# sjtuytc/betapose

Hardware: AMD Instinct MI355X
Metric: frames/sec (640x480, 50-kp KPD) (higher is better)
Workload: dtype f32 as an exact 3-way bf16 operand split (6 bf16 MFMA products), f32 accumulate and activations

## Files before the change

betapose_amd/_lib.py:

```python
from __future__ import annotations

import ctypes as C
import os
import threading

_HERE = os.path.dirname(os.path.abspath(__file__))
LIB_PATH = os.environ.get("BP_LIB") or os.path.join(_HERE, "libbetapose_hip.so")
_lock = threading.Lock()
_lib = None

c_float_p = C.POINTER(C.c_float)
c_double_p = C.POINTER(C.c_double)
c_int_p = C.POINTER(C.c_int)
vp = C.c_void_p

PROTOTYPES = {
    "bp_last_error": (C.c_char_p, []),
    "bp_version": (C.c_int, []),
    "bp_device_count": (C.c_int, []),
    "bp_device_name": (C.c_int, [C.c_int, C.c_char_p, C.c_int]),
    "bp_yolo_create": (C.c_int, [C.c_char_p, C.c_char_p, C.c_int, C.c_int, C.c_int, C.POINTER(vp)]),
    "bp_yolo_create_from_memory": (C.c_int, [C.c_char_p, vp, C.c_size_t, C.c_int, C.c_int, C.c_int, C.POINTER(vp)]),
    "bp_yolo_clone": (C.c_int, [vp, C.POINTER(vp)]),
    "bp_kpd_clone": (C.c_int, [vp, C.POINTER(vp)]),
    "bp_yolo_destroy": (None, [vp]),
    "bp_yolo_rows": (C.c_int, [vp]),
    "bp_yolo_attrs": (C.c_int, [vp]),
    "bp_yolo_forward": (C.c_int, [vp, vp, C.c_int, vp, vp]),
    "bp_yolo_forward_select": (C.c_int, [vp, vp, C.c_int, C.c_float, C.c_int, vp, vp, vp]),
    "bp_yolo_select": (C.c_int, [vp, C.c_int, C.c_int, C.c_int, C.c_float, C.c_int, vp, vp]),
    "bp_yolo_tap_count": (C.c_int, [vp]),
    "bp_yolo_tap_info": (C.c_int, [vp, C.c_int, C.c_char_p, C.c_int, c_int_p, c_int_p, c_int_p]),
    "bp_yolo_tap_copy": (C.c_int, [vp, C.c_int, C.c_int, vp, vp]),
    "bp_kpd_create": (C.c_int, [vp, C.c_size_t, C.c_int, C.c_int, C.c_int, C.POINTER(vp)]),
    "bp_kpd_destroy": (None, [vp]),
    "bp_kpd_forward": (C.c_int, [vp, vp, C.c_int, vp, vp]),
    "bp_kpd_forward_argmax": (C.c_int, [vp, vp, C.c_int, vp, vp, vp]),
    "bp_kpd_tap_count": (C.c_int, [vp]),
    "bp_kpd_tap_info": (C.c_int, [vp, C.c_int, C.c_char_p, C.c_int, c_int_p, c_int_p, c_int_p]),
    "bp_kpd_tap_copy": (C.c_int, [vp, C.c_int, C.c_int, vp, vp]),
    "bp_yolo_set_policy": (C.c_int, [vp, C.c_int, C.c_int, C.c_int, C.c_int]),
    "bp_kpd_set_policy": (C.c_int, [vp, C.c_int, C.c_int, C.c_int, C.c_int]),
    "bp_yolo_set_precision": (C.c_int, [vp, C.c_int]),
    "bp_kpd_set_precision": (C.c_int, [vp, C.c_int]),
    "bp_calibrate_ticks": (C.c_int, [C.c_longlong, c_float_p, vp]),
    "bp_yolo_set_prefetch": (C.c_int, [vp, C.c_int]),
    "bp_kpd_set_prefetch": (C.c_int, [vp, C.c_int]),
    "bp_yolo_set_fusion": (C.c_int, [vp, C.c_int]),
    "bp_kpd_set_fusion": (C.c_int, [vp, C.c_int]),
    "bp_yolo_fused_launches": (C.c_int, [vp, C.c_int, C.POINTER(C.c_int)]),
    "bp_kpd_fused_launches": (C.c_int, [vp, C.c_int, C.POINTER(C.c_int)]),
    "bp_yolo_xcd_errors": (C.c_int, [vp, C.POINTER(C.c_int), vp]),
    "bp_kpd_xcd_errors": (C.c_int, [vp, C.POINTER(C.c_int), vp]),
# ... 129 lines not shown
```

betapose_amd/csrc/aux_kernels.hip:

```cpp
#include "bp_common.h"

namespace bp {

__device__ __forceinline__ void store_plane(unsigned short* planes, long long idx, long long plane_elems, int np, float v) {
    if (np == 1) {
        const _Float16 h = (_Float16)v;
        planes[idx] = __builtin_bit_cast(unsigned short, h);
    } else if (np == 3) {
        const __bf16 h1 = (__bf16)v;
        const float r1 = v - (float)h1;
        const __bf16 h2 = (__bf16)r1;
        const __bf16 h3 = (__bf16)(r1 - (float)h2);
        planes[idx] = __builtin_bit_cast(unsigned short, h1);
        planes[idx + plane_elems] = __builtin_bit_cast(unsigned short, h2);
        planes[idx + 2 * plane_elems] = __builtin_bit_cast(unsigned short, h3);
    }
}

static inline int grid_for(long long n, int block = 256, int cap = 4096) {
    BP_CHECK(n < (1ll << 31), "tensor too large for 32-bit indexing");
    long long g = (n + block - 1) / block;
    return (int)(g < 1 ? 1 : (g > cap ? cap : g));
}

// ... 221 lines not shown
}

struct YoloHeads {
    YoloHead h[4];
    int n;
};
__device__ __forceinline__ float sigmoidf_(float x) { return 1.f / (1.f + expf(-x)); }

__global__ void yolo_decode_kernel(YoloHeads hs, int N, int reso, int attrs, int rows, float* __restrict__ pred) {
    const long long total = (long long)N * rows;
    for (int e = blockIdx.x * blockDim.x + threadIdx.x; e < (int)total; e += gridDim.x * blockDim.x) {
        const int row = (int)(e % rows);
        const int n = (int)(e / rows);
        int hi = 0;
        for (int k = 1; k < hs.n; ++k)
            if (row >= hs.h[k].row_off) hi = k;
        const YoloHead& H = hs.h[hi];
        const int g = H.g;
        const int r = row - H.row_off;
        const int a = r / (g * g);
        const int cell = r - a * g * g;
        const int gy = cell / g, gx = cell - gy * g;
        const float stride = (float)(reso / g);
        const float* t = H.t + ((long long)n * g * g + cell) * (3 * attrs) + a * attrs;
        float* o = pred + e * attrs;
        o[0] = (sigmoidf_(t[0]) + (float)gx) * stride;
        o[1] = (sigmoidf_(t[1]) + (float)gy) * stride;
        o[2] = (expf(t[2]) * (H.aw[a] / stride)) * stride;
        o[3] = (expf(t[3]) * (H.ah[a] / stride)) * stride;
        for (int k = 4; k < attrs; ++k) o[k] = sigmoidf_(t[k]);
    }
}
void launch_yolo_decode(const YoloHead* heads, int nheads, int N, int reso, int attrs, int rows, float* pred,
                        hipStream_t s) {
    BP_CHECK(nheads <= 4, "at most 4 yolo heads");
    YoloHeads hs;
    hs.n = nheads;
    for (int i = 0; i < nheads; ++i) hs.h[i] = heads[i];
    hipLaunchKernelGGL(yolo_decode_kernel, dim3(grid_for((long long)N * rows)), dim3(256), 0, s, hs, N, reso, attrs, rows, pred);
}

__global__ __launch_bounds__(1024) void yolo_select_kernel(const float* __restrict__ pred, int rows, int attrs,
                                                            float conf, int num_classes, float* __restrict__ sel, int sel_ld) {
    __shared__ float sv[16];
    __shared__ int si[16];
    const int n = blockIdx.x;
    const float* P = pred + (long long)n * rows * attrs;
// ... 24 lines not shown
            if (sv[k] > best || (sv[k] == best && si[k] < bi)) { best = sv[k]; bi = si[k]; }
        float* o = sel + (long long)n * sel_ld;
        if (best < 0.f) {
            o[0] = __int_as_float(-1);
            for (int k = 1; k < 8; ++k) o[k] = 0.f;
        } else {
            const float* q = P + (long long)bi * attrs;
            o[0] = __int_as_float(bi);
            o[1] = q[0] - q[2] / 2;
            o[2] = q[1] - q[3] / 2;
            o[3] = q[0] + q[2] / 2;
            o[4] = q[1] + q[3] / 2;
            o[5] = q[4];
            o[6] = q[5];
            o[7] = 0.f;
        }
    }
}
void launch_yolo_select(const float* pred, int N, int rows, int attrs, float conf, int num_classes, float* sel,
                        hipStream_t s, int sel_ld) {
    hipLaunchKernelGGL(yolo_select_kernel, dim3(N), dim3(1024), 0, s, pred, rows, attrs, conf, num_classes, sel, sel_ld);
}

__global__ __launch_bounds__(1024) void yolo_decode_select_kernel(YoloHeads hs, int reso, int attrs, int rows, float conf, int num_classes,
                                                                   float* __restrict__ sel, int sel_ld) {
    __shared__ float sv[16];
    __shared__ int si[16];
    const int n = blockIdx.x;
    const int ncls = min(num_classes, attrs - 5);
    auto locate = [&](int row, int* a) -> const float* {
        int hi = 0;
        for (int k = 1; k < hs.n; ++k)
            if (row >= hs.h[k].row_off) hi = k;
        const YoloHead& H = hs.h[hi];
        const int g = H.g, r = row - H.row_off;
        *a = r / (g * g);
        const int cell = r - *a * g * g;
        return H.t + ((long long)n * g * g + cell) * (3 * attrs) + *a * attrs;
    };
    float best = -1.f;
    int bi = 0x7fffffff;
    for (int r = threadIdx.x; r < rows; r += blockDim.x) {
        int a;
        const float* t = locate(r, &a);
        const float obj = sigmoidf_(t[4]);
        if (!(obj > conf)) continue;
        int cls = 0;
        float cm = sigmoidf_(t[5]);
        for (int k = 1; k < ncls; ++k) {
            const float v = sigmoidf_(t[5 + k]);
            if (v > cm) { cm = v; cls = k; }
        }
        if (cls != 0) continue;
        if (obj > best || (obj == best && r < bi)) { best = obj; bi = r; }
    }
    for (int off = 32; off > 0; off >>= 1) {
        const float ov = __shfl_down(best, off, 64);
        const int oi = __shfl_down(bi, off, 64);
        if (ov > best || (ov == best && oi < bi)) { best = ov; bi = oi; }
    }
    const int w = threadIdx.x >> 6;
    if ((threadIdx.x & 63) == 0) { sv[w] = best; si[w] = bi; }
    __syncthreads();
    if (threadIdx.x == 0) {
        for (int k = 1; k < (int)(blockDim.x >> 6); ++k)
            if (sv[k] > best || (sv[k] == best && si[k] < bi)) { best = sv[k]; bi = si[k]; }
        float* o = sel + (long long)n * sel_ld;
        if (best < 0.f) {
            o[0] = __int_as_float(-1);
            for (int k = 1; k < 8; ++k) o[k] = 0.f;
        } else {
            int a, hi = 0;
            const float* t = locate(bi, &a);
            for (int k = 1; k < hs.n; ++k)
                if (bi >= hs.h[k].row_off) hi = k;
            const YoloHead& H = hs.h[hi];
            const int g = H.g, r = bi - H.row_off, cell = r - a * g * g;
            const int gy = cell / g, gx = cell - gy * g;
            const float stride = (float)(reso / g);
            const float q0 = (sigmoidf_(t[0]) + (float)gx) * stride;
            const float q1 = (sigmoidf_(t[1]) + (float)gy) * stride;
            const float q2 = (expf(t[2]) * (H.aw[a] / stride)) * stride;
            const float q3 = (expf(t[3]) * (H.ah[a] / stride)) * stride;
            o[0] = __int_as_float(bi);
            o[1] = q0 - q2 / 2;
            o[2] = q1 - q3 / 2;
            o[3] = q0 + q2 / 2;
            o[4] = q1 + q3 / 2;
            o[5] = sigmoidf_(t[4]);
            o[6] = sigmoidf_(t[5]);
            o[7] = 0.f;
        }
    }
}
void launch_yolo_decode_select(const YoloHead* heads, int nheads, int N, int reso, int attrs, int rows, float conf, int num_classes,
                               float* sel, hipStream_t s, int sel_ld) {
    BP_CHECK(nheads <= 4, "at most 4 yolo heads");
    YoloHeads hs;
    hs.n = nheads;
    for (int i = 0; i < nheads; ++i) hs.h[i] = heads[i];
    hipLaunchKernelGGL(yolo_decode_select_kernel, dim3(N), dim3(1024), 0, s, hs, reso, attrs, rows, conf, num_classes, sel, sel_ld);
}

__global__ __launch_bounds__(256) void heatmap_argmax_kernel(const float* __restrict__ hm, int H, int W,
                                                              float* __restrict__ out, int C, int out_ld) {
    __shared__ float sv[4];
    __shared__ int si[4];
    const int HW = H * W;
    const float* P = hm + (long long)blockIdx.x * HW;
    float best = -INFINITY;
    int bi = 0x7fffffff;
    for (int i = threadIdx.x; i < HW; i += 256) {
        const float v = P[i];
        if (v > best) { best = v; bi = i; }
    }
    for (int off = 32; off > 0; off >>= 1) {
        const float ov = __shfl_down(best, off, 64);
        const int oi = __shfl_down(bi, off, 64);
        if (ov > best || (ov == best && oi < bi)) { best = ov; bi = oi; }
    }
    if ((threadIdx.x & 63) == 0) { sv[threadIdx.x >> 6] = best; si[threadIdx.x >> 6] = bi; }
    __syncthreads();
    if (threadIdx.x == 0) {
        for (int k = 1; k < 4; ++k)
// ... 261 lines not shown
```

betapose_amd/csrc/bp_common.h:

```cpp
#pragma once
#include <hip/hip_runtime.h>
#include <cstdint>
#include <cstdio>
#include <mutex>
#include <set>
#include <stdexcept>
#include <string>
#include <utility>

namespace bp {

struct Error : std::runtime_error {
    using std::runtime_error::runtime_error;
};

#define BP_HIP(expr)                                                                      \
    do {                                                                                  \
        hipError_t _e = (expr);                                                           \
        if (_e != hipSuccess)                                                             \
            throw ::bp::Error(std::string(#expr) + ": " + hipGetErrorString(_e) + " @" +  \
                              __FILE__ + ":" + std::to_string(__LINE__));                 \
    } while (0)

#define BP_CHECK(cond, msg)                                                               \
// ... 178 lines not shown
};

size_t mega_lds_bytes(const MegaOp& o);
void mega_make_conv_op(const ConvParams& p, int tile, MegaOp* out);
void launch_mega(const MegaArgs& a, size_t lds_bytes, hipStream_t s);

void launch_nchw_to_nhwc(const float* in, float* out, int N, int C, int H, int W, hipStream_t s);
void launch_nhwc_to_nchw(const float* in, int in_ld, float* out, int N, int C, int H, int W, hipStream_t s);
void launch_maxpool3s2p1(const float* in, float* out, int N, int H, int W, int C, int OH, int OW, hipStream_t s,
                         unsigned short* planes = nullptr, long long plane_elems = 0, int np = 0);
void launch_add(const float* a, int a_ld, const float* b, int b_ld, float* out, int out_ld,
                long long pixels, int C, hipStream_t s);
void launch_upsample2(const float* in, int in_ld, float* out, int out_ld, int N, int H, int W, int C, hipStream_t s);
void launch_copy_channels(const float* in, int in_ld, float* out, int out_ld, long long pixels, int C, hipStream_t s);
void launch_pixel_shuffle2(const float* in, float* out, int N, int H, int W, int C, hipStream_t s,
                           unsigned short* planes = nullptr, long long plane_elems = 0, int np = 0);
int avgpool_parts(int HW);
void launch_avgpool(const float* in, int in_ld, float* out, int N, int HW, int C, hipStream_t s);
void launch_fc(const float* in, const float* w, const float* bias, float* out, int N, int Cin, int Cout,
               int act, int in_parts, float in_scale, hipStream_t s);

struct YoloHead {
    const float* t;
    int g;
    float aw[3], ah[3];
    int row_off;
};
void launch_yolo_decode(const YoloHead* heads, int nheads, int N, int reso, int attrs, int rows,
                        float* pred, hipStream_t s);
void launch_yolo_select(const float* pred, int N, int rows, int attrs, float conf, int num_classes,
                        float* sel, hipStream_t s, int sel_ld = 8);
void launch_yolo_decode_select(const YoloHead* heads, int nheads, int N, int reso, int attrs, int rows, float conf, int num_classes,
                               float* sel, hipStream_t s, int sel_ld = 8);
void launch_heatmap_argmax(const float* hm, int N, int C, int H, int W, float* out, hipStream_t s, int out_ld = 0);

void launch_f32_to_f16(const float* in, unsigned short* out, long long n, hipStream_t s);
void launch_f32_to_bf16x3(const float* in, unsigned short* out_planes, long long n, hipStream_t s);
void launch_f32_to_f16_staged(const float* in, unsigned short* out, int CoutPad, int Kpad, hipStream_t s);
void launch_f32_to_bf16x3_staged(const float* in, unsigned short* out, int CoutPad, int Kpad, hipStream_t s, int Cin_pl = 0);
void launch_probe_placement(int* d_out, int blocks, hipStream_t s);
void launch_spin_ticks(long long ticks, hipStream_t s);

void launch_crop(const uint8_t* frames, int batch, int H, int W, const float* sel, int reso, const float* boxes,
                 float* out_nhwc, float* out_nchw, float* pts, int oh, int ow, hipStream_t s, int sel_ld = 8, int pts_ld = 8);

struct ResizeTables {
    const int* hb;
    const int* hk;
    int ksize_h;
    const int* vb;
    const int* vk;
    int ksize_v;
};
void launch_resize_bicubic(const uint8_t* in, int batch, int H, int W, uint8_t* tmp, float* out_nhwc, uint8_t* out_u8,
                           int oh, int ow, const ResizeTables& t, int swap_rb, hipStream_t s);

// ... 2 lines not shown
```

betapose_amd/csrc/c_api.cpp:

```cpp
#include "../../include/betapose_hip.h"

#include <algorithm>
#include <cmath>
#include <cstdlib>
#include <cstring>
#include <fstream>
#include <memory>
#include <sstream>
#include <vector>

#include "engine.h"
#include "frame_io.h"

namespace bp {
int solve_pnp(const double* P, const double* U, int n, const double* K, double* R, double* t);
int solve_pnp_refined(const double* P, const double* U, int n, const double* K, double* R, double* t);
int solve_pnp_ransac(const double* P, const double* U, int n, const double* K, double reproj_err, int max_trials,
                     double confidence, double* R, double* t, unsigned char* inlier_mask);
void pnp_ransac_samples(int n, int max_trials, int* idx);
void pnp_ransac_trials_needed(int n, double confidence, int* need);
int pose_nms(const float* bboxes, const float* bbox_scores, const float* preds, const float* scores, int n, int K,
             int* out_pick, float* out_pose, float* out_score, float* out_prop);
int pose_error_blocks(int n);
void launch_pose_errors(const double* model, int n, const double* gt, const double* est, int P, const double* K,
// ... 255 lines not shown
    y->net->forward(d_img, false, batch, d_pred, 0.f, 0, nullptr, (hipStream_t)stream);
    return 0;
    BP_CATCH
}
int bp_yolo_forward_select(bp_yolo* y, const float* d_img, int batch, float conf, int num_classes, float* d_pred,
                           float* d_sel, void* stream) {
    BP_TRY
    BP_CHECK(y && d_img && d_sel, "null argument");
    y->net->forward(d_img, false, batch, d_pred, conf, num_classes, d_sel, (hipStream_t)stream);
    return 0;
    BP_CATCH
}

int bp_yolo_select(const float* d_pred, int batch, int rows, int attrs, float conf, int num_classes, float* d_sel,
                   void* stream) {
    BP_TRY
    BP_CHECK(d_pred && d_sel && batch >= 1 && rows >= 1 && attrs >= 6, "bad argument");
    bp::launch_yolo_select(d_pred, batch, rows, attrs, conf, num_classes, d_sel, (hipStream_t)stream);
    BP_HIP(hipGetLastError());
    return 0;
    BP_CATCH
}

static int tap_info(const bp::Net& n, int i, char* name, int cap, int* C, int* H, int* W) {
    if (i < 0 || i >= n.tap_count()) { g_err = "tap index"; return -1; }
    if (name && cap > 0) std::snprintf(name, cap, "%s", n.tap_name(i));
    n.tap_shape(i, C, H, W);
    return 0;
}
int bp_yolo_tap_count(const bp_yolo* y) { return y ? y->net->tap_count() : -1; }
int bp_yolo_tap_info(const bp_yolo* y, int i, char* name, int cap, int* C, int* H, int* W) {
    if (!y || !C || !H || !W) { g_err = "null argument"; return -1; }
    return tap_info(*y->net, i, name, cap, C, H, W);
}
int bp_yolo_tap_copy(bp_yolo* y, int i, int batch, float* d_out, void* stream) {
    BP_TRY
    BP_CHECK(y && d_out, "null argument");
    y->net->tap_copy(i, batch, d_out, (hipStream_t)stream);
    return 0;
    BP_CATCH
}

int bp_kpd_create(const float* stream, size_t n_floats, int n_classes, int max_batch, int device, bp_kpd** out) {
    BP_TRY
    BP_CHECK(stream && out, "null argument");
    BP_HIP(hipSetDevice(device));
// ... 143 lines not shown
int bp_yolo_xcd_errors(bp_yolo* y, int* count, void* stream) {
    BP_TRY
    BP_CHECK(y && count, "null argument");
    BP_HIP(hipSetDevice(y->device));
    *count = y->net->take_xcd_errors((hipStream_t)stream);
    return 0;
    BP_CATCH
}
int bp_kpd_xcd_errors(bp_kpd* k, int* count, void* stream) {
    BP_TRY
    BP_CHECK(k && count, "null argument");
    BP_HIP(hipSetDevice(k->device));
    *count = k->net->take_xcd_errors((hipStream_t)stream);
    return 0;
    BP_CATCH
}
int bp_yolo_set_stamps(bp_yolo* y, unsigned long long* d_buf, int slots) { y->net->set_stamps(d_buf, slots); return 0; }
int bp_kpd_set_stamps(bp_kpd* k, unsigned long long* d_buf, int slots) { k->net->set_stamps(d_buf, slots); return 0; }
static int op_name(const bp::Net& net, int i, char* out, int cap) {
    if (i < 0 || i >= (int)net.ops().size() || !out || cap <= 0) return -1;
    const bp::Op& op = net.ops()[i];
    if (op.type == bp::OP_CONV)
        std::snprintf(out, (size_t)cap, "%s k%d %dx%d %d->%d s%d", net.op_name(i), op.conv.ksize, op.conv.OH, op.conv.OW, op.conv.Cin,
                      op.conv.Cout, op.conv.stride);
    else
        std::snprintf(out, (size_t)cap, "%s", net.op_name(i));
    return op.type == bp::OP_CONV ? 1 : 0;
}
int bp_yolo_op_name(const bp_yolo* y, int i, char* out, int cap) { return op_name(*y->net, i, out, cap); }
int bp_kpd_op_name(const bp_kpd* k, int i, char* out, int cap) { return op_name(*k->net, i, out, cap); }
size_t bp_yolo_device_bytes(const bp_yolo* y) { return y->net->device_bytes(); }
size_t bp_kpd_device_bytes(const bp_kpd* k) { return k->net->device_bytes(); }

int bp_crop(const uint8_t* d_frames, int batch, int H, int W, const float* d_sel, int reso, const float* d_boxes,
            float* d_out_nchw, float* d_out_nhwc, float* d_pts, int oh, int ow, void* stream) {
    BP_TRY
    BP_CHECK(d_frames && (d_sel || d_boxes) && (d_out_nchw || d_out_nhwc), "null argument");
    bp::launch_crop(d_frames, batch, H, W, d_sel, reso, d_boxes, d_out_nhwc, d_out_nchw, d_pts, oh, ow, (hipStream_t)stream);
    BP_HIP(hipGetLastError());
    return 0;
    BP_CATCH
}

int bp_resize_bicubic(const uint8_t* d_in, int batch, int H, int W, int oh, int ow, int swap_rb, uint8_t* d_out_u8,
                      float* d_out_nhwc, void* stream) {
    BP_TRY
    BP_CHECK(d_in && (d_out_u8 || d_out_nhwc), "null argument");
// ... 722 lines not shown
```

betapose_amd/csrc/engine.cpp:

```cpp
#include "engine.h"

#include <algorithm>
#include <cmath>
#include <cstdlib>
#include <cstring>
#include <sstream>

namespace bp {

Arena::~Arena() {
    for (void* p : ptrs_) (void)hipFree(p);
}
void* Arena::alloc_bytes(size_t bytes) {
    void* p = nullptr;
    bytes = (bytes + 255) & ~size_t(255);
    BP_HIP(hipMalloc(&p, bytes));
    ptrs_.push_back(p);
    total_ += bytes;
    return p;
}
float* Arena::alloc(size_t n) { return static_cast<float*>(alloc_bytes(n * sizeof(float))); }

Tensor Net::new_tensor(int H, int W, int C) {
    Tensor t;
// ... 556 lines not shown
        dB = upload_weights(B.data(), B.size());
    }

    Op op;
    op.type = OP_CONV;
    op.name = name;
    ConvParams& c = op.conv;
    c.in = in.p; c.in_ld = in.ld; c.N = 1; c.H = in.H; c.W = in.W; c.Cin = Cin;
    c.w = dW; c.Kpad = Kpad; c.Ktrue = K; c.bias = dB; c.cin_pack = cpk;
    c.out = out_view.p; c.out_ld = out_view.ld; c.OH = OH; c.OW = OW; c.Cout = Cout;
    c.ksize = k; c.stride = stride; c.pad = pad; c.act = act;
    c.res = res ? res->p : nullptr; c.res_ld = res ? res->ld : 0; c.res_scale = res_scale;
    c.res_after_act = res_after_act; c.store_mode = store_mode;
    c.M = OH * OW; c.nchunks = Kpad / 32; c.splits = 1; c.chunks_per_split = c.nchunks; c.partial = nullptr;
    c.tickets = nullptr;
    c.stamps = nullptr;
    c.w16 = nullptr; c.w16s = nullptr;
    c.in16 = nullptr; c.out16 = nullptr; c.wpl = nullptr; c.wbd = nullptr; c.in16_plane = c.out16_plane = 0; c.out_np = 0; c.abl = 0; c.skip_f32 = 0; c.res16 = nullptr; c.net_prec = PREC_F32;
    c.pool_out = nullptr; c.hy_full = c.hy_splits = c.hy_cps = 0;
    c.pf_ptr = nullptr; c.xcd_home = 0; c.xcc_of = nullptr; c.err_word = nullptr; c.tickets_local = nullptr; c.mtiles = c.n_tiles = c.work_blocks = c.pf_first = 0;
    c.pf_ntn = c.pf_splits = c.pf_cps = c.pf_nchunks = c.pf_tile_stride = c.pf_chunk_bytes = c.pf_cap = 0;
    c.CoutPad = CoutPad;
    const double Kalg = (double)k * k * Cin;
    op.flops = 2.0 * OH * OW * (double)Cout * Kalg;
    op.bytes = 4.0 * ((double)Cout * Kalg + (double)in.H * in.W * Cin + (double)OH * OW * Cout + (res ? (double)OH * OW * Cout : 0.0));
    ops_.push_back(op);
    return (int)ops_.size() - 1;
}

size_t Net::workspace_need() const {
    size_t need = 0;
    for (const Op& op : ops_) {
        if (op.type != OP_CONV) continue;
        for (int lone = 0; lone < 2; ++lone)
            for (int b = 1; b <= max_batch_; ++b) {
                int tile, splits, cps;
                choose_launch(op, b, force_tile_, sk_target_, sk_min_chunks_, 64, &tile, &splits, &cps, lone != 0);
                ConvParams q = op.conv; q.N = b; q.M = b * q.OH * q.OW; q.splits = splits;
                if (splits > 1) {
                    need = std::max(need, (size_t)splits * conv_tiles(q, tile) * conv_tile_bm(tile) * conv_tile_bn(tile));
                } else {
                    int full = 0, hs = 0, hcps = 0;
                    if (conv_hybrid_plan(q, tile, (size_t)-1, &full, &hs, &hcps))
                        need = std::max(need, (size_t)hs * (conv_tiles(q, tile) - full) * conv_tile_bm(tile) * conv_tile_bn(tile));
                }
            }
// ... 695 lines not shown
    }
    std::vector<Tensor> T(n);
    std::vector<char> has(n, 0);
    in_nhwc_ = arena_.alloc((size_t)max_batch * reso * reso * 3);
    std::vector<std::pair<int, int>> copy_members;
    for (int i = 0; i < n; ++i) {
        if (members[i].empty()) continue;
        T[i] = new_tensor(shp[i].H, shp[i].W, shp[i].C);
        has[i] = 1;
        int off = 0;
        for (int m : members[i]) {
            const bool producible = L[m].type == "convolutional" || L[m].type == "shortcut" || L[m].type == "upsample";
            if (!has[m] && producible && members[m].empty()) {
                T[m] = T[i];
                T[m].p = T[i].p + off;
                T[m].C = shp[m].C;
                has[m] = 1;
            } else {
                copy_members.push_back({i, m});
            }
            off += shp[m].C;
        }
    }
    for (int i = 0; i < n; ++i) {
        if (has[i] || alias[i] != i) continue;
        if (L[i].type == "convolutional" && fused_into[i] >= 0) continue;
        T[i] = new_tensor(shp[i].H, shp[i].W, shp[i].C);
        has[i] = 1;
    }
    auto tensor_of = [&](int i) -> const Tensor& {
        const int r = alias[i];
        BP_CHECK(has[r], "internal: tensor not materialised");
        return T[r];
    };
    size_t cur = 0;
    auto take = [&](size_t cnt) {
        BP_CHECK(cur + cnt <= n_floats, "weights stream too short for this cfg");
        const float* p = stream + cur;
        cur += cnt;
        return p;
    };
    Tensor input;
    input.p = in_nhwc_; input.H = reso; input.W = reso; input.C = 3; input.ld = 3;
    int row_off = 0;
    for (int i = 0; i < n; ++i) {
        const CfgBlock& b = L[i];
        if (b.type == "convolutional") {
            const Tensor& in = i ? tensor_of(i - 1) : input;
            const int k = b.geti("size", 1), st = b.geti("stride", 1);
            const int pad = b.has("pad") && !b.gets("pad").empty() ? (k - 1) / 2 : 0;
            const int Cout = shp[i].C, Cin = in.C;
            ConvWeights cw;
            if (b.geti("batch_normalize", 0) > 0) {
                cw.bn_bias = take(Cout); cw.bn_scale = take(Cout); cw.bn_mean = take(Cout); cw.bn_var = take(Cout);
            } else {
                cw.bias = take(Cout);
            }
            cw.w = take((size_t)Cout * Cin * k * k);
            const std::string a = b.gets("activation");
            const int act = a == "leaky" ? ACT_LEAKY : (a == "relu" ? ACT_RELU : ACT_LINEAR);
            BP_CHECK(a == "leaky" || a == "linear" || a == "relu", "unsupported activation " + a);
            int mode = ST_NHWC;
            const Tensor* res = nullptr;
            int dst = i;
            if (fused_into[i] >= 0) {
                dst = fused_into[i];
                if (L[dst].type == "shortcut") res = &tensor_of(dst + L[dst].geti("from", -3));
                else mode = ST_UP2;
            }
            add_conv("conv" + std::to_string(i), in, T[alias[dst]], cw, Cout, k, st, pad, act, mode, res, nullptr,
                     1, 1e-5f, shp[i].H, shp[i].W);
            add_tap(std::to_string(dst), T[alias[dst]]);
        } else if (b.type == "shortcut") {
            if (fused_from[i] >= 0) continue;
            const Tensor& a = tensor_of(i - 1);
            const Tensor& c = tensor_of(i + b.geti("from", -3));
            Op op; op.type = OP_ADD; op.name = "shortcut" + std::to_string(i);
            op.a = a.p; op.a_ld = a.ld; op.b = c.p; op.b_ld = c.ld; op.out = T[i].p; op.out_ld = T[i].ld;
            op.H = shp[i].H; op.W = shp[i].W; op.C = shp[i].C;
            ops_.push_back(op);
            add_tap(std::to_string(i), T[i]);
        } else if (b.type == "upsample") {
            if (fused_from[i] >= 0) continue;
            const Tensor& a = tensor_of(i - 1);
            Op op; op.type = OP_UPSAMPLE; op.name = "upsample" + std::to_string(i);
            op.a = a.p; op.a_ld = a.ld; op.out = T[i].p; op.out_ld = T[i].ld;
            op.H = a.H; op.W = a.W; op.C = a.C;
            ops_.push_back(op);
            add_tap(std::to_string(i), T[i]);
        } else if (b.type == "route") {
            if (members[i].empty()) continue;
            int off = 0;
            for (int m : members[i]) {
                for (auto& cm : copy_members)
                    if (cm.first == i && cm.second == m) {
                        Op op; op.type = OP_COPYCH; op.name = "concat" + std::to_string(i);
                        op.a = T[m].p; op.a_ld = T[m].ld; op.out = T[i].p + off; op.out_ld = T[i].ld;
                        op.H = shp[i].H; op.W = shp[i].W; op.C = shp[m].C;
                        ops_.push_back(op);
                    }
                off += shp[m].C;
            }
            add_tap(std::to_string(i), T[i]);
        } else if (b.type == "yolo") {
            const Tensor& t = tensor_of(i - 1);
            std::vector<int> mask = parse_ints(b.gets("mask"));
            std::vector<int> an = parse_ints(b.gets("anchors"));
            const int classes = b.geti("classes", 1);
            BP_CHECK(mask.size() == 3, "yolo layer needs 3 masked anchors");
            BP_CHECK(t.C == 3 * (5 + classes) && t.ld == t.C, "yolo head channel count");
            BP_CHECK(attrs_ == 0 || attrs_ == 5 + classes, "heads disagree on classes");
            attrs_ = 5 + classes;
            YoloHead h{};
            h.t = t.p; h.g = t.H; h.row_off = row_off;
            for (int a = 0; a < 3; ++a) {
                BP_CHECK(mask[a] >= 0 && 2 * mask[a] + 1 < (int)an.size(), "anchor mask");
                h.aw[a] = (float)an[2 * mask[a]];
                h.ah[a] = (float)an[2 * mask[a] + 1];
            }
            heads_.push_back(h);
            row_off += 3 * t.H * t.W;
        }
    }
    BP_CHECK(!heads_.empty() && heads_.size() <= 4, "cfg must have 1..4 yolo layers");
    rows_ = row_off;
    pred_ = arena_.alloc((size_t)max_batch * rows_ * attrs_);
    finalize();
}

void YoloNet::forward(const float* d_img, bool nhwc_input, int batch, float* d_pred, float conf, int num_classes,
                      float* d_sel, hipStream_t s, int sel_ld) {
    BP_CHECK(batch >= 1 && batch <= max_batch_, "batch out of range");
    if (nhwc_input) {
        if (d_img != in_nhwc_)
            BP_HIP(hipMemcpyAsync(in_nhwc_, d_img, (size_t)batch * reso_ * reso_ * 3 * sizeof(float),
                                  hipMemcpyDeviceToDevice, s));
    } else {
        launch_nchw_to_nhwc(d_img, in_nhwc_, batch, 3, reso_, reso_, s);
    }
    run_ops(batch, s);
    static const bool two_kernels = std::getenv("BP_NO_DECODE_FUSION") != nullptr;
    if (d_sel && !d_pred && !two_kernels) {
        launch_yolo_decode_select(heads_.data(), (int)heads_.size(), batch, reso_, attrs_, rows_, conf, num_classes, d_sel, s, sel_ld);
    } else {
        float* pred = d_pred ? d_pred : pred_;
        launch_yolo_decode(heads_.data(), (int)heads_.size(), batch, reso_, attrs_, rows_, pred, s);
        if (d_sel) launch_yolo_select(pred, batch, rows_, attrs_, conf, num_classes, d_sel, s, sel_ld);
    }
    BP_HIP(hipGetLastError());
}

KpdNet::KpdNet(const float* stream, size_t n_floats, int n_classes, int max_batch, int inH, int inW,
               std::shared_ptr<WeightStore> store)
    : Net(max_batch, store), n_floats_(n_floats), n_classes_(n_classes), inH_(inH), inW_(inW) {
    BP_CHECK(inH % 32 == 0 && inW % 32 == 0, "KPD input must be a multiple of 32");
    BP_CHECK(n_classes >= 1, "n_classes");
    outC_ = std::min(n_classes, 50);
    size_t cur = 0;
    auto take = [&](size_t cnt) {
        BP_CHECK(cur + cnt <= n_floats, "KPD stream too short");
        const float* p = stream + cur;
        cur += cnt;
        return p;
    };
    auto take_conv_bn = [&](int cout, int cin, int k) {
        ConvWeights cw;
// ... 160 lines not shown
```

betapose_amd/csrc/engine.h:

```cpp
#pragma once
#include <map>
#include <memory>
#include <mutex>
#include <string>
#include <vector>

#include "bp_common.h"

namespace bp {

struct Tensor {
    float* p = nullptr;
    int H = 0, W = 0, C = 0;
    int ld = 0;
};

class Arena {
public:
    ~Arena();
    float* alloc(size_t n_floats);
    void* alloc_bytes(size_t bytes);
    size_t total_bytes() const { return total_; }
private:
    std::vector<void*> ptrs_;
    size_t total_ = 0;
};

enum OpType : int {
    OP_CONV, OP_MAXPOOL, OP_ADD, OP_UPSAMPLE, OP_COPYCH, OP_PIXSHUF, OP_AVGPOOL, OP_FC
};

struct Op {
    OpType type;
    ConvParams conv{};
    int tile = TILE_64x64;
    const float* a = nullptr; int a_ld = 0;
    const float* b = nullptr; int b_ld = 0;
    float* out = nullptr; int out_ld = 0;
    int H = 0, W = 0, C = 0, OH = 0, OW = 0;
    const float* w = nullptr; const float* bias = nullptr; int Cin = 0, Cout = 0, act = 0;
    int in_parts = 1; float in_scale = 1.f;
    float* pool_out = nullptr;
    unsigned short* out16 = nullptr; long long out16_plane = 0;
    std::string name;
    double flops = 0;
    double bytes = 0;
};

struct ConvWeights {
    const float* w = nullptr;
    const float* bn_bias = nullptr, *bn_scale = nullptr, *bn_mean = nullptr, *bn_var = nullptr;
    const float* bias = nullptr;
};

struct WeightStore {
    Arena arena;
    std::vector<float*> ptrs;
    std::map<const float*, unsigned short*> f16;
    std::map<const float*, unsigned short*> bf16x3;
    std::map<const float*, unsigned short*> bf16x3s;
    std::map<const float*, unsigned short*> f16s;
    std::map<const float*, unsigned short*> wbd3;
    std::map<const float*, unsigned short*> wpl1, wpl3;
    std::mutex f16_mutex;
};

class Net {
// ... 80 lines not shown
    void run_op_unfused(const Op& op, int batch, hipStream_t s);
    bool f16_res_ = false;
    unsigned plan_version_ = 0;
};

class YoloNet : public Net {
public:
    YoloNet(const std::string& cfg_text, const float* stream, size_t n_floats, int reso, int max_batch,
            std::shared_ptr<WeightStore> store = nullptr, bool darknet_bn = false);
    YoloNet* clone() const { return new YoloNet(cfg_text_, nullptr, n_floats_, reso_, max_batch_, store_, darknet_bn_); }
    int rows() const { return rows_; }
    int attrs() const { return attrs_; }
    int reso() const { return reso_; }
    void forward(const float* d_img, bool nhwc_input, int batch, float* d_pred, float conf, int num_classes,
                 float* d_sel, hipStream_t s, int sel_ld = 8);
    float* input_nhwc() { return in_nhwc_; }
    float* pred_buffer() { return pred_; }
private:
    std::string cfg_text_;
    size_t n_floats_ = 0;
    int reso_, rows_ = 0, attrs_ = 0;
    float* in_nhwc_ = nullptr;
    float* pred_ = nullptr;
    std::vector<YoloHead> heads_;
};

class KpdNet : public Net {
public:
    KpdNet(const float* stream, size_t n_floats, int n_classes, int max_batch, int inH = 320, int inW = 256,
           std::shared_ptr<WeightStore> store = nullptr);
    KpdNet* clone() const { return new KpdNet(nullptr, n_floats_, n_classes_, max_batch_, inH_, inW_, store_); }
    int out_c() const { return outC_; }
    int out_h() const { return inH_ / 4; }
    int out_w() const { return inW_ / 4; }
    int in_h() const { return inH_; }
    int in_w() const { return inW_; }
    void forward(const float* d_inps, bool nhwc_input, int batch, float* d_hm, float* d_kp, hipStream_t s, int kp_ld = 0);
    float* input_nhwc() { return in_nhwc_; }
private:
    size_t n_floats_ = 0;
    int n_classes_ = 0;
    int inH_, inW_, outC_;
    float* in_nhwc_ = nullptr;
    float* hm_ = nullptr;
    int hm_op_ = -1;
};
// ... 9 lines not shown
```

betapose_amd/yolo_util.py:

```python
from __future__ import annotations

from . import _lib
from .darknet import sel_to_dets


def write_results(prediction, confidence, num_classes, nms=True, nms_conf=0.4):
    import torch
    _lib.require_gpu()
    pred = prediction if prediction.is_cuda else prediction.cuda()
    pred = pred.contiguous().float()
    B, rows, attrs = pred.shape
    sel = torch.empty((B, 8), device=pred.device, dtype=torch.float32)
    _lib.check(_lib.lib().bp_yolo_select(pred.data_ptr(), B, rows, attrs, float(confidence), int(num_classes),
                                         sel.data_ptr(), _lib.current_stream()))
    return sel_to_dets(sel)


def dynamic_write_results(prediction, confidence, num_classes, nms=True, nms_conf=0.4):
    return write_results(prediction, confidence, num_classes, nms, nms_conf)
```

include/betapose_hip.h:

```cpp
#ifndef BETAPOSE_HIP_H
#define BETAPOSE_HIP_H

#include <stddef.h>
#include <stdint.h>

#ifdef __cplusplus
extern "C" {
#endif

typedef struct bp_yolo bp_yolo;
typedef struct bp_kpd bp_kpd;
typedef struct bp_pipeline bp_pipeline;

#define BP_RESULT_FLOATS 316
#define BP_KP_FLOATS 6
#define BP_SEL_FLOATS 8

#define BP_POSE_DOUBLES 166
#define BP_PNP_MAX_POINTS 64

const char* bp_last_error(void);
int bp_version(void);
int bp_device_count(void);
int bp_device_name(int device, char* out, int cap);

int bp_yolo_create(const char* cfg_path, const char* weights_path, int reso, int max_batch, int device, bp_yolo** out);
int bp_yolo_create_from_memory(const char* cfg_text, const float* stream, size_t n_floats, int reso, int max_batch,
                               int device, bp_yolo** out);
int bp_yolo_clone(const bp_yolo* y, bp_yolo** out);
void bp_yolo_destroy(bp_yolo* y);
int bp_yolo_rows(const bp_yolo* y);
int bp_yolo_attrs(const bp_yolo* y);
int bp_yolo_forward(bp_yolo* y, const float* d_img_nchw, int batch, float* d_pred, void* stream);
int bp_yolo_forward_select(bp_yolo* y, const float* d_img_nchw, int batch, float conf, int num_classes, float* d_pred,
                           float* d_sel, void* stream);
int bp_yolo_select(const float* d_pred, int batch, int rows, int attrs, float conf, int num_classes, float* d_sel,
                   void* stream);
int bp_yolo_tap_count(const bp_yolo* y);
int bp_yolo_tap_info(const bp_yolo* y, int i, char* name, int cap, int* C, int* H, int* W);
int bp_yolo_tap_copy(bp_yolo* y, int i, int batch, float* d_out_nchw, void* stream);

int bp_kpd_create(const float* stream, size_t n_floats, int n_classes, int max_batch, int device, bp_kpd** out);
int bp_kpd_clone(const bp_kpd* k, bp_kpd** out);
void bp_kpd_destroy(bp_kpd* k);
int bp_kpd_forward(bp_kpd* k, const float* d_inps_nchw, int batch, float* d_hm, void* stream);
int bp_kpd_forward_argmax(bp_kpd* k, const float* d_inps_nchw, int batch, float* d_hm, float* d_kp, void* stream);
int bp_kpd_tap_count(const bp_kpd* k);
int bp_kpd_tap_info(const bp_kpd* k, int i, char* name, int cap, int* C, int* H, int* W);
int bp_kpd_tap_copy(bp_kpd* k, int i, int batch, float* d_out_nchw, void* stream);

int bp_yolo_set_policy(bp_yolo* y, int sk_target_blocks, int sk_min_chunks, int sk_max_splits, int force_tile);
int bp_kpd_set_policy(bp_kpd* k, int sk_target_blocks, int sk_min_chunks, int sk_max_splits, int force_tile);
int bp_yolo_set_precision(bp_yolo* y, int precision);
int bp_kpd_set_precision(bp_kpd* k, int precision);
int bp_yolo_op_stats(const bp_yolo* y, double* flops, double* bytes, int cap);
int bp_kpd_op_stats(const bp_kpd* k, double* flops, double* bytes, int cap);
int bp_yolo_profile(bp_yolo* y, int batch, int iters, float* ms, int* info, int cap, void* stream);
int bp_calibrate_ticks(long long ticks, float* ms, void* stream);
int bp_yolo_set_prefetch(bp_yolo* y, int on);
int bp_kpd_set_prefetch(bp_kpd* k, int on);
// ... 108 lines not shown
```

Before: 1010.

## Split YOLO decode-select across many blocks and pad head conv channels

The fused decode+select kernel now launches a 2-D grid of 256-row blocks per image instead of one 1024-thread block per image. Partial argmaxes are combined through a ticket atomic, and the last block finishes the reduction and writes the selection. YOLO head conv outputs with channel counts not divisible by 4 are stored with a padded leading dimension, presumably so the conv kernel can use aligned stores. This adds a workspace, an atomic last-block reduction and an ld field threaded through the decode paths. A new C API exposes decode-select on external head tensors.

```diff
diff --git a/betapose_amd/_lib.py b/betapose_amd/_lib.py
--- a/betapose_amd/_lib.py
+++ b/betapose_amd/_lib.py
@@ -29,6 +29,9 @@
     "bp_yolo_forward": (C.c_int, [vp, vp, C.c_int, vp, vp]),
     "bp_yolo_forward_select": (C.c_int, [vp, vp, C.c_int, C.c_float, C.c_int, vp, vp, vp]),
     "bp_yolo_select": (C.c_int, [vp, C.c_int, C.c_int, C.c_int, C.c_float, C.c_int, vp, vp]),
+    "bp_yolo_select_ws_ints": (C.c_size_t, [C.c_int, C.c_int]),
+    "bp_yolo_decode_select": (C.c_int, [C.POINTER(vp), c_int_p, c_int_p, c_float_p, C.c_int, C.c_int, C.c_int, C.c_int, C.c_float, C.c_int,
+                                        vp, vp, vp, vp]),
     "bp_yolo_tap_count": (C.c_int, [vp]),
     "bp_yolo_tap_info": (C.c_int, [vp, C.c_int, C.c_char_p, C.c_int, c_int_p, c_int_p, c_int_p]),
     "bp_yolo_tap_copy": (C.c_int, [vp, C.c_int, C.c_int, vp, vp]),
diff --git a/betapose_amd/csrc/aux_kernels.hip b/betapose_amd/csrc/aux_kernels.hip
--- a/betapose_amd/csrc/aux_kernels.hip
+++ b/betapose_amd/csrc/aux_kernels.hip
@@ -267,7 +267,7 @@
         const int cell = r - a * g * g;
         const int gy = cell / g, gx = cell - gy * g;
         const float stride = (float)(reso / g);
-        const float* t = H.t + ((long long)n * g * g + cell) * (3 * attrs) + a * attrs;
+        const float* t = H.t + ((long long)n * g * g + cell) * H.ld + a * attrs;
         float* o = pred + e * attrs;
         o[0] = (sigmoidf_(t[0]) + (float)gx) * stride;
         o[1] = (sigmoidf_(t[1]) + (float)gy) * stride;
@@ -338,11 +338,22 @@
     hipLaunchKernelGGL(yolo_select_kernel, dim3(N), dim3(1024), 0, s, pred, rows, attrs, conf, num_classes, sel, sel_ld);
 }
 
-__global__ __launch_bounds__(1024) void yolo_decode_select_kernel(YoloHeads hs, int reso, int attrs, int rows, float conf, int num_classes,
-                                                                   float* __restrict__ sel, int sel_ld) {
-    __shared__ float sv[16];
-    __shared__ int si[16];
-    const int n = blockIdx.x;
+static constexpr int SEL_ROWS = 256;
+int yolo_select_blocks(int rows) { return (rows + SEL_ROWS - 1) / SEL_ROWS; }
+size_t yolo_select_ws_ints(int N, int rows) { return (size_t)N * (1 + 2 * (size_t)yolo_select_blocks(rows)); }
+
+__device__ __forceinline__ bool sel_better(float ov, int oi, float best, int bi) { return ov > best || (ov == best && oi < bi); }
+
+__global__ __launch_bounds__(SEL_ROWS) void yolo_decode_select_kernel(YoloHeads hs, int reso, int attrs, int rows, float conf, int num_classes,
+                                                                      float* __restrict__ sel, int sel_ld, int* __restrict__ ws) {
+    __shared__ float sv[SEL_ROWS / 64];
+    __shared__ int si[SEL_ROWS / 64];
+    __shared__ int s_last;
+    const int n = blockIdx.y;
+    const int nblk = gridDim.x;
+    int* ticket = ws + (long long)n * (1 + 2 * nblk);
+    float* part_v = reinterpret_cast<float*>(ticket + 1);
+    int* part_i = ticket + 1 + nblk;
     const int ncls = min(num_classes, attrs - 5);
     auto locate = [&](int row, int* a) -> const float* {
         int hi = 0;
@@ -352,35 +363,63 @@
         const int g = H.g, r = row - H.row_off;
         *a = r / (g * g);
         const int cell = r - *a * g * g;
-        return H.t + ((long long)n * g * g + cell) * (3 * attrs) + *a * attrs;
+        return H.t + ((long long)n * g * g + cell) * H.ld + *a * attrs;
     };
     float best = -1.f;
     int bi = 0x7fffffff;
-    for (int r = threadIdx.x; r < rows; r += blockDim.x) {
+    const int r = blockIdx.x * SEL_ROWS + threadIdx.x;
+    if (r < rows) {
         int a;
         const float* t = locate(r, &a);
         const float obj = sigmoidf_(t[4]);
-        if (!(obj > conf)) continue;
-        int cls = 0;
-        float cm = sigmoidf_(t[5]);
-        for (int k = 1; k < ncls; ++k) {
-            const float v = sigmoidf_(t[5 + k]);
-            if (v > cm) { cm = v; cls = k; }
-        }
-        if (cls != 0) continue;
-        if (obj > best || (obj == best && r < bi)) { best = obj; bi = r; }
+        if (obj > conf) {
+            int cls = 0;
+            float cm = sigmoidf_(t[5]);
+            for (int k = 1; k < ncls; ++k) {
+                const float v = sigmoidf_(t[5 + k]);
+                if (v > cm) { cm = v; cls = k; }
+            }
+            if (cls == 0) { best = obj; bi = r; }
+        }
     }
     for (int off = 32; off > 0; off >>= 1) {
         const float ov = __shfl_down(best, off, 64);
         const int oi = __shfl_down(bi, off, 64);
-        if (ov > best || (ov == best && oi < bi)) { best = ov; bi = oi; }
+        if (sel_better(ov, oi, best, bi)) { best = ov; bi = oi; }
     }
     const int w = threadIdx.x >> 6;
     if ((threadIdx.x & 63) == 0) { sv[w] = best; si[w] = bi; }
     __syncthreads();
     if (threadIdx.x == 0) {
-        for (int k = 1; k < (int)(blockDim.x >> 6); ++k)
-            if (sv[k] > best || (sv[k] == best && si[k] < bi)) { best = sv[k]; bi = si[k]; }
+        for (int k = 1; k < SEL_ROWS / 64; ++k)
+            if (sel_better(sv[k], si[k], best, bi)) { best = sv[k]; bi = si[k]; }
+        int last = 1;
+        if (nblk > 1) {
+            part_v[blockIdx.x] = best;
+            part_i[blockIdx.x] = bi;
+            const int tk = __hip_atomic_fetch_add(ticket, 1, __ATOMIC_ACQ_REL, __HIP_MEMORY_SCOPE_AGENT);
+            last = tk == nblk - 1;
+            if (last) __hip_atomic_store(ticket, 0, __ATOMIC_RELAXED, __HIP_MEMORY_SCOPE_AGENT);
+        }
+        s_last = last;
+    }
+    __syncthreads();
+    if (!s_last || threadIdx.x >= 64) return;
+    if (nblk > 1) {
+        best = -1.f;
+        bi = 0x7fffffff;
+        for (int k = threadIdx.x; k < nblk; k += 64) {
+            const float ov = __hip_atomic_load(&part_v[k], __ATOMIC_RELAXED, __HIP_MEMORY_SCOPE_AGENT);
+            const int oi = __hip_atomic_load(&part_i[k], __ATOMIC_RELAXED, __HIP_MEMORY_SCOPE_AGENT);
+            if (sel_better(ov, oi, best, bi)) { best = ov; bi = oi; }
+        }
+        for (int off = 32; off > 0; off >>= 1) {
+            const float ov = __shfl_down(best, off, 64);
+            const int oi = __shfl_down(bi, off, 64);
+            if (sel_better(ov, oi, best, bi)) { best = ov; bi = oi; }
+        }
+    }
+    if (threadIdx.x == 0) {
         float* o = sel + (long long)n * sel_ld;
         if (best < 0.f) {
             o[0] = __int_as_float(-1);
@@ -391,7 +430,7 @@
             for (int k = 1; k < hs.n; ++k)
                 if (bi >= hs.h[k].row_off) hi = k;
             const YoloHead& H = hs.h[hi];
-            const int g = H.g, r = bi - H.row_off, cell = r - a * g * g;
+            const int g = H.g, rr = bi - H.row_off, cell = rr - a * g * g;
             const int gy = cell / g, gx = cell - gy * g;
             const float stride = (float)(reso / g);
             const float q0 = (sigmoidf_(t[0]) + (float)gx) * stride;
@@ -410,12 +449,14 @@
     }
 }
 void launch_yolo_decode_select(const YoloHead* heads, int nheads, int N, int reso, int attrs, int rows, float conf, int num_classes,
-                               float* sel, hipStream_t s, int sel_ld) {
+                               float* sel, hipStream_t s, int sel_ld, int* ws) {
     BP_CHECK(nheads <= 4, "at most 4 yolo heads");
+    BP_CHECK(ws != nullptr, "yolo_decode_select needs its ticket / partial workspace");
     YoloHeads hs;
     hs.n = nheads;
     for (int i = 0; i < nheads; ++i) hs.h[i] = heads[i];
-    hipLaunchKernelGGL(yolo_decode_select_kernel, dim3(N), dim3(1024), 0, s, hs, reso, attrs, rows, conf, num_classes, sel, sel_ld);
+    hipLaunchKernelGGL(yolo_decode_select_kernel, dim3(yolo_select_blocks(rows), N), dim3(SEL_ROWS), 0, s, hs, reso, attrs, rows, conf,
+                       num_classes, sel, sel_ld, ws);
 }
 
 __global__ __launch_bounds__(256) void heatmap_argmax_kernel(const float* __restrict__ hm, int H, int W,
diff --git a/betapose_amd/csrc/bp_common.h b/betapose_amd/csrc/bp_common.h
--- a/betapose_amd/csrc/bp_common.h
+++ b/betapose_amd/csrc/bp_common.h
@@ -224,6 +224,7 @@
 
 struct YoloHead {
     const float* t;
+    int ld;
     int g;
     float aw[3], ah[3];
     int row_off;
@@ -232,8 +233,10 @@
                         float* pred, hipStream_t s);
 void launch_yolo_select(const float* pred, int N, int rows, int attrs, float conf, int num_classes,
                         float* sel, hipStream_t s, int sel_ld = 8);
+int yolo_select_blocks(int rows);
+size_t yolo_select_ws_ints(int N, int rows);
 void launch_yolo_decode_select(const YoloHead* heads, int nheads, int N, int reso, int attrs, int rows, float conf, int num_classes,
-                               float* sel, hipStream_t s, int sel_ld = 8);
+                               float* sel, hipStream_t s, int sel_ld, int* ws);
 void launch_heatmap_argmax(const float* hm, int N, int C, int H, int W, float* out, hipStream_t s, int out_ld = 0);
 
 void launch_f32_to_f16(const float* in, unsigned short* out, long long n, hipStream_t s);
diff --git a/betapose_amd/csrc/c_api.cpp b/betapose_amd/csrc/c_api.cpp
--- a/betapose_amd/csrc/c_api.cpp
+++ b/betapose_amd/csrc/c_api.cpp
@@ -301,6 +301,32 @@
     BP_CATCH
 }
 
+size_t bp_yolo_select_ws_ints(int batch, int rows) { return batch >= 1 && rows >= 1 ? bp::yolo_select_ws_ints(batch, rows) : 0; }
+
+int bp_yolo_decode_select(const float* const* d_heads, const int* grid, const int* ld, const float* anchors, int nheads, int batch,
+                          int reso, int attrs, float conf, int num_classes, float* d_pred, float* d_sel, int* d_ws, void* stream) {
+    BP_TRY
+    BP_CHECK(d_heads && grid && ld && anchors && d_sel && (d_pred || d_ws), "null argument");
+    BP_CHECK(nheads >= 1 && nheads <= 4 && batch >= 1 && attrs >= 6 && reso >= 1, "bad argument");
+    bp::YoloHead h[4];
+    int rows = 0;
+    for (int i = 0; i < nheads; ++i) {
+        BP_CHECK(d_heads[i] && grid[i] >= 1 && reso / grid[i] >= 1 && ld[i] >= 3 * attrs, "bad head");
+        h[i].t = d_heads[i]; h[i].ld = ld[i]; h[i].g = grid[i]; h[i].row_off = rows;
+        for (int a = 0; a < 3; ++a) { h[i].aw[a] = anchors[(i * 3 + a) * 2]; h[i].ah[a] = anchors[(i * 3 + a) * 2 + 1]; }
+        rows += 3 * grid[i] * grid[i];
+    }
+    if (d_pred) {
+        bp::launch_yolo_decode(h, nheads, batch, reso, attrs, rows, d_pred, (hipStream_t)stream);
+        bp::launch_yolo_select(d_pred, batch, rows, attrs, conf, num_classes, d_sel, (hipStream_t)stream);
+    } else {
+        bp::launch_yolo_decode_select(h, nheads, batch, reso, attrs, rows, conf, num_classes, d_sel, (hipStream_t)stream, 8, d_ws);
+    }
+    BP_HIP(hipGetLastError());
+    return 0;
+    BP_CATCH
+}
+
 static int tap_info(const bp::Net& n, int i, char* name, int cap, int* C, int* H, int* W) {
     if (i < 0 || i >= n.tap_count()) { g_err = "tap index"; return -1; }
     if (name && cap > 0) std::snprintf(name, cap, "%s", n.tap_name(i));
@@ -490,7 +516,7 @@
     const bp::Op& op = net.ops()[i];
     if (op.type == bp::OP_CONV)
         std::snprintf(out, (size_t)cap, "%s k%d %dx%d %d->%d s%d", net.op_name(i), op.conv.ksize, op.conv.OH, op.conv.OW, op.conv.Cin,
-                      op.conv.Cout, op.conv.stride);
+                      op.cout, op.conv.stride);
     else
         std::snprintf(out, (size_t)cap, "%s", net.op_name(i));
     return op.type == bp::OP_CONV ? 1 : 0;
diff --git a/betapose_amd/csrc/engine.cpp b/betapose_amd/csrc/engine.cpp
--- a/betapose_amd/csrc/engine.cpp
+++ b/betapose_amd/csrc/engine.cpp
@@ -602,6 +602,7 @@
     c.pf_ntn = c.pf_splits = c.pf_cps = c.pf_nchunks = c.pf_tile_stride = c.pf_chunk_bytes = c.pf_cap = 0;
     c.CoutPad = CoutPad;
     const double Kalg = (double)k * k * Cin;
+    op.cout = Cout;
     op.flops = 2.0 * OH * OW * (double)Cout * Kalg;
     op.bytes = 4.0 * ((double)Cout * Kalg + (double)in.H * in.W * Cin + (double)OH * OW * Cout + (res ? (double)OH * OW * Cout : 0.0));
     ops_.push_back(op);
@@ -1343,10 +1344,19 @@
             off += shp[m].C;
         }
     }
+    const bool head_generic = std::getenv("BP_HEAD_GENERIC") != nullptr;
+    std::vector<char> head_pad(n, 0);
     for (int i = 0; i < n; ++i) {
         if (has[i] || alias[i] != i) continue;
         if (L[i].type == "convolutional" && fused_into[i] >= 0) continue;
-        T[i] = new_tensor(shp[i].H, shp[i].W, shp[i].C);
+        const bool head = L[i].type == "convolutional" && i + 1 < n && L[i + 1].type == "yolo" && cons[i].size() == 1 && cons[i][0] == i + 1;
+        if (head && (shp[i].C & 3) != 0 && !head_generic) {
+            T[i] = new_tensor(shp[i].H, shp[i].W, round_up(shp[i].C, 4));
+            T[i].C = shp[i].C;
+            head_pad[i] = 1;
+        } else {
+            T[i] = new_tensor(shp[i].H, shp[i].W, shp[i].C);
+        }
         has[i] = 1;
     }
     auto tensor_of = [&](int i) -> const Tensor& {
@@ -1391,6 +1401,7 @@
             }
             add_conv("conv" + std::to_string(i), in, T[alias[dst]], cw, Cout, k, st, pad, act, mode, res, nullptr,
                      1, 1e-5f, shp[i].H, shp[i].W);
+            if (head_pad[i]) ops_.back().conv.Cout = T[i].ld;
             add_tap(std::to_string(dst), T[alias[dst]]);
         } else if (b.type == "shortcut") {
             if (fused_from[i] >= 0) continue;
@@ -1429,11 +1440,11 @@
             std::vector<int> an = parse_ints(b.gets("anchors"));
             const int classes = b.geti("classes", 1);
             BP_CHECK(mask.size() == 3, "yolo layer needs 3 masked anchors");
-            BP_CHECK(t.C == 3 * (5 + classes) && t.ld == t.C, "yolo head channel count");
+            BP_CHECK(t.C == 3 * (5 + classes) && t.ld >= t.C, "yolo head channel count");
             BP_CHECK(attrs_ == 0 || attrs_ == 5 + classes, "heads disagree on classes");
             attrs_ = 5 + classes;
             YoloHead h{};
-            h.t = t.p; h.g = t.H; h.row_off = row_off;
+            h.t = t.p; h.ld = t.ld; h.g = t.H; h.row_off = row_off;
             for (int a = 0; a < 3; ++a) {
                 BP_CHECK(mask[a] >= 0 && 2 * mask[a] + 1 < (int)an.size(), "anchor mask");
                 h.aw[a] = (float)an[2 * mask[a]];
@@ -1446,6 +1457,9 @@
     BP_CHECK(!heads_.empty() && heads_.size() <= 4, "cfg must have 1..4 yolo layers");
     rows_ = row_off;
     pred_ = arena_.alloc((size_t)max_batch * rows_ * attrs_);
+    const size_t sel_ints = yolo_select_ws_ints(max_batch, rows_);
+    sel_ws_ = (int*)arena_.alloc_bytes(sel_ints * sizeof(int));
+    BP_HIP(hipMemset(sel_ws_, 0, sel_ints * sizeof(int)));
     finalize();
 }
 
@@ -1462,7 +1476,7 @@
     run_ops(batch, s);
     static const bool two_kernels = std::getenv("BP_NO_DECODE_FUSION") != nullptr;
     if (d_sel && !d_pred && !two_kernels) {
-        launch_yolo_decode_select(heads_.data(), (int)heads_.size(), batch, reso_, attrs_, rows_, conf, num_classes, d_sel, s, sel_ld);
+        launch_yolo_decode_select(heads_.data(), (int)heads_.size(), batch, reso_, attrs_, rows_, conf, num_classes, d_sel, s, sel_ld, sel_ws_);
     } else {
         float* pred = d_pred ? d_pred : pred_;
         launch_yolo_decode(heads_.data(), (int)heads_.size(), batch, reso_, attrs_, rows_, pred, s);
diff --git a/betapose_amd/csrc/engine.h b/betapose_amd/csrc/engine.h
--- a/betapose_amd/csrc/engine.h
+++ b/betapose_amd/csrc/engine.h
@@ -43,6 +43,7 @@
     float* pool_out = nullptr;
     unsigned short* out16 = nullptr; long long out16_plane = 0;
     std::string name;
+    int cout = 0;
     double flops = 0;
     double bytes = 0;
 };
@@ -169,6 +170,7 @@
     int reso_, rows_ = 0, attrs_ = 0;
     float* in_nhwc_ = nullptr;
     float* pred_ = nullptr;
+    int* sel_ws_ = nullptr;
     std::vector<YoloHead> heads_;
 };
 
diff --git a/betapose_amd/yolo_util.py b/betapose_amd/yolo_util.py
--- a/betapose_amd/yolo_util.py
+++ b/betapose_amd/yolo_util.py
@@ -18,3 +18,33 @@
 
 def dynamic_write_results(prediction, confidence, num_classes, nms=True, nms_conf=0.4):
     return write_results(prediction, confidence, num_classes, nms, nms_conf)
+
+
+def select_workspace(batch, rows, device):
+    import torch
+    n = int(_lib.lib().bp_yolo_select_ws_ints(int(batch), int(rows)))
+    return torch.zeros(n, device=device, dtype=torch.int32)
+
+
+def decode_select_heads(heads, anchors, reso, attrs, confidence, num_classes, two_kernels=False, ws=None):
+    import ctypes as C
+    import numpy as np
+    import torch
+    _lib.require_gpu()
+    n, B, dev = len(heads), heads[0].shape[0], heads[0].device
+    for h in heads:
+        if not (h.is_cuda and h.is_contiguous() and h.dtype == torch.float32 and h.dim() == 4 and h.shape[0] == B and h.shape[1] == h.shape[2]):
+            raise ValueError("heads must be contiguous f32 device tensors [B, g, g, ld]")
+    grid = (C.c_int * n)(*[int(h.shape[1]) for h in heads])
+    ld = (C.c_int * n)(*[int(h.shape[3]) for h in heads])
+    ptrs = (C.c_void_p * n)(*[h.data_ptr() for h in heads])
+    an = np.ascontiguousarray(anchors, dtype=np.float32).reshape(n, 3, 2)
+    rows = sum(3 * int(h.shape[1]) ** 2 for h in heads)
+    sel = torch.empty((B, 8), device=dev, dtype=torch.float32)
+    pred = torch.empty((B, rows, attrs), device=dev, dtype=torch.float32) if two_kernels else None
+    if not two_kernels and ws is None:
+        ws = select_workspace(B, rows, dev)
+    _lib.check(_lib.lib().bp_yolo_decode_select(ptrs, grid, ld, an.ctypes.data_as(_lib.c_float_p), n, B, int(reso), int(attrs), float(confidence),
+                                                int(num_classes), pred.data_ptr() if two_kernels else None, sel.data_ptr(),
+                                                None if two_kernels else ws.data_ptr(), _lib.current_stream()))
+    return (sel, pred) if two_kernels else sel
diff --git a/include/betapose_hip.h b/include/betapose_hip.h
--- a/include/betapose_hip.h
+++ b/include/betapose_hip.h
@@ -36,6 +36,9 @@
                            float* d_sel, void* stream);
 int bp_yolo_select(const float* d_pred, int batch, int rows, int attrs, float conf, int num_classes, float* d_sel,
                    void* stream);
+size_t bp_yolo_select_ws_ints(int batch, int rows);
+int bp_yolo_decode_select(const float* const* d_heads, const int* grid, const int* ld, const float* anchors, int nheads, int batch,
+                          int reso, int attrs, float conf, int num_classes, float* d_pred, float* d_sel, int* d_ws, void* stream);
 int bp_yolo_tap_count(const bp_yolo* y);
 int bp_yolo_tap_info(const bp_yolo* y, int i, char* name, int cap, int* C, int* H, int* W);
 int bp_yolo_tap_copy(bp_yolo* y, int i, int batch, float* d_out_nchw, void* stream);
```

Result: no change. 1014, median of 4 (+0.4%).
